# atomicarchitects/equiformer

Measured on NVIDIA H100. Metric: edges/sec fwd+bwd, QM9 Lmax=2 batch, higher is better.
Workload: dtype f32

## Files before the change

equiformer_b200/csrc/eqf_gemm_tf32x3.cu:

```cuda
#include <cuda.h>
#include <cuda_runtime.h>

#include <cstdint>
#include <cstdlib>
#include <mutex>
#include <string>

#include "eqf_common.cuh"
#include "eqf_tc.cuh"

namespace eqf {
namespace tf32x3 {

using namespace tc;

constexpr int BM = 128;
constexpr int BK = kKTile;
constexpr int kRowBytes = BK * 4;
constexpr int kThreads = 384;
constexpr int kConsumerWarps = 8, kConsumerThreads = kConsumerWarps * 32;
constexpr int kSmemBudget = 227 * 1024;
constexpr int kMaxStages = 8;

template <int BN>
struct Smem {
  static constexpr int kABytes = BM * kRowBytes;
  static constexpr int kBBytes = BN * kRowBytes;
  static constexpr int kStageBytes = kABytes + 2 * kBBytes;
  static constexpr int kStagesRaw = (kSmemBudget - 2048) / kStageBytes;
  static constexpr int kStages = kStagesRaw > kMaxStages ? kMaxStages : kStagesRaw;
  static_assert(kStages >= 2, "tile does not fit shared memory");
  static constexpr int kTotal = kStages * kStageBytes + 1024  + 1024 ;
};

struct Params {
  float* C;
  long long M, ldc;
  long long n_tiles;
  int n_blocks;
  int N, K;
};

template <int BN>
__global__ void __launch_bounds__(kThreads, 1)
gemm_tf32x3_kernel(const __grid_constant__ CUtensorMap map_a, const __grid_constant__ CUtensorMap map_bhi,
                   const __grid_constant__ CUtensorMap map_blo, Params p) {
  using S = Smem<BN>;
  constexpr int kStages = S::kStages;
  extern __shared__ uint8_t smem_raw[];
  uint8_t* smem = reinterpret_cast<uint8_t*>((reinterpret_cast<uintptr_t>(smem_raw) + 1023) & ~uintptr_t(1023));
  uint64_t* full = reinterpret_cast<uint64_t*>(smem + kStages * S::kStageBytes);
  uint64_t* empty = full + kStages;

  const int warp = threadIdx.x >> 5, lane = threadIdx.x & 31, wg = warp >> 2;
  const int k_tiles = (p.K + BK - 1) / BK;
  if (threadIdx.x == 0) {
    for (int s = 0; s < kStages; ++s) { mbar_init(&full[s], 1); mbar_init(&empty[s], kConsumerWarps); }
    asm volatile("fence.mbarrier_init.release.cluster;" ::: "memory");
  }
  __syncthreads();

  if (wg == 0) {
    reg_dealloc<40>();
    if (threadIdx.x == 0) {
      prefetch_map(&map_a); prefetch_map(&map_bhi); prefetch_map(&map_blo);
      int s = 0;
      uint32_t ph = 0;
      for (long long tile = blockIdx.x; tile < p.n_tiles; tile += gridDim.x) {
        const int m0 = (int)(tile / p.n_blocks) * BM;
        const int n0 = (int)(tile % p.n_blocks) * BN;
        for (int kt = 0; kt < k_tiles; ++kt) {
          mbar_wait_hint(&empty[s], ph ^ 1);
          uint8_t* st = smem + s * S::kStageBytes;
          mbar_expect_tx(&full[s], (uint32_t)S::kStageBytes);
          tma_load_2d(st, &map_a, kt * BK, m0, &full[s]);
          tma_load_2d(st + S::kABytes, &map_bhi, kt * BK, n0, &full[s]);
          tma_load_2d(st + S::kABytes + S::kBBytes, &map_blo, kt * BK, n0, &full[s]);
          if (++s == kStages) { s = 0; ph ^= 1; }
        }
      }
    }
  } else {
    reg_alloc<232>();
    const int row_wg = (wg - 1) * 64 + (warp & 3) * 16;
    int s = 0;
    uint32_t ph = 0;
    for (long long tile = blockIdx.x; tile < p.n_tiles; tile += gridDim.x) {
      const long long m0 = (tile / p.n_blocks) * BM;
      const int n0 = (int)(tile % p.n_blocks) * BN;
      float acc[BN / 2], part[BN / 2];
#pragma unroll
      for (int i = 0; i < BN / 2; ++i) acc[i] = 0.f;
      for (int kt = 0; kt < k_tiles; ++kt) {
        mbar_wait_hint(&full[s], ph);
        const uint32_t st = smem_u32(smem + s * S::kStageBytes);
        uint32_t hi[16], lo[16];
        load_a_split(st, row_wg, lane, hi, lo);
#pragma unroll
        for (int i = 0; i < BN / 2; ++i) part[i] = 0.f;
        mma_ktile_3xtf32<BN>(part, hi, lo, st + S::kABytes, st + S::kABytes + S::kBBytes);
        wgmma_wait<0>();
        __syncwarp();
        if (lane == 0) mbar_arrive(&empty[s]);
#pragma unroll
        for (int i = 0; i < BN / 2; ++i) acc[i] += part[i];
        if (++s == kStages) { s = 0; ph ^= 1; }
      }
      store_acc<BN>(acc, p.C, p.ldc, m0 + row_wg, p.M, n0, p.N, lane, false);
    }
  }
}

__global__ void split_kernel(const float* __restrict__ w, float* __restrict__ hi, float* __restrict__ lo, long long n) {
  for (long long i = (long long)blockIdx.x * blockDim.x + threadIdx.x; i < n; i += (long long)gridDim.x * blockDim.x) {
    const float v = w[i];
    const float h = tf32_rn(v);
    hi[i] = h;
    lo[i] = tf32_rn(v - h);
  }
}

__global__ void split_transpose_kernel(const float* __restrict__ w, long long ldw, float* __restrict__ hi,
                                       float* __restrict__ lo, long long N, long long K) {
  const long long n_el = N * K;
  for (long long i = (long long)blockIdx.x * blockDim.x + threadIdx.x; i < n_el; i += (long long)gridDim.x * blockDim.x) {
    const long long n = i / K, k = i - n * K;
    const float v = w[k * ldw + n];
    const float h = tf32_rn(v);
    hi[i] = h;
    lo[i] = tf32_rn(v - h);
  }
}

template <int BN>
static int launch(const CUtensorMap& ma, const CUtensorMap& mh, const CUtensorMap& ml, const Params& p, long long m_blocks,
                  int n_blocks, cudaStream_t s) {
  static std::once_flag once;
  static cudaError_t attr_err = cudaSuccess;
  std::call_once(once, [] {
    attr_err = cudaFuncSetAttribute(gemm_tf32x3_kernel<BN>, cudaFuncAttributeMaxDynamicSharedMemorySize, Smem<BN>::kTotal);
  });
  if (attr_err != cudaSuccess) return check_cuda(attr_err, "gemm_tf32x3 smem attribute");
  Params q = p;
  q.n_blocks = n_blocks;
  q.n_tiles = m_blocks * n_blocks;
  const long long sms = device_sms();
  const unsigned grid = (unsigned)(q.n_tiles < sms ? q.n_tiles : sms);
  gemm_tf32x3_kernel<BN><<<grid, kThreads, Smem<BN>::kTotal, s>>>(ma, mh, ml, q);
  return check_cuda(cudaGetLastError(), "gemm_tf32x3_kernel launch");
}

namespace wg {

constexpr int BKR = BK;
constexpr int kBoxBytes = BKR * 128;
constexpr int kMaxBN = 128;

struct WParams {
  float* out;
  long long R, rows_per_slice, K1;
  int N;
  int reduce;
};

template <int BN>
struct WSmem {
  static constexpr int kABytes = (BM / 32) * kBoxBytes;
  static constexpr int kGRawBytes = BKR * BN * 4;
  static constexpr int kGBytes = BN * kRowBytes;
  static constexpr int kStageBytes = kABytes + kGRawBytes + 2 * kGBytes;
  static constexpr int kStagesRaw = (kSmemBudget - 2048) / kStageBytes;
  static constexpr int kStages = kStagesRaw > kMaxStages ? kMaxStages : kStagesRaw;
  static_assert(kStages >= 2, "tile does not fit shared memory");
  static constexpr int kTotal = kStages * kStageBytes + 1024 + 1024;
};

__device__ __forceinline__ void load_at_split(uint32_t tile, int row0, int lane, uint32_t (&hi)[16], uint32_t (&lo)[16]) {
  const int g = row0 + (lane >> 2), t = lane & 3;
#pragma unroll
  for (int kb = 0; kb < BKR / 8; ++kb) {
#pragma unroll
    for (int q = 0; q < 4; ++q) {
      const int m = g + ((q & 1) ? 8 : 0);
      const int r = kb * 8 + t + ((q & 2) ? 4 : 0);
      const int c = m & 31;
      const uint32_t addr = tile + (uint32_t)(m >> 5) * kBoxBytes + (uint32_t)r * 128u + (uint32_t)((((c >> 2) ^ (r & 7)) << 4) + (c & 3) * 4);
      const float x = lds32(addr);
      const float h = tf32_rn_fast(x);
      hi[kb * 4 + q] = __float_as_uint(h);
      lo[kb * 4 + q] = __float_as_uint(tf32_rn_fast(x - h));
    }
  }
}

template <int BN>
__global__ void __launch_bounds__(kThreads, 1)
wgrad_tf32x3_kernel(const __grid_constant__ CUtensorMap map_a, const __grid_constant__ CUtensorMap map_g, WParams p) {
  using S = WSmem<BN>;
  constexpr int kStages = S::kStages;
  extern __shared__ uint8_t smem_raw[];
  uint8_t* smem = reinterpret_cast<uint8_t*>((reinterpret_cast<uintptr_t>(smem_raw) + 1023) & ~uintptr_t(1023));
  uint64_t* full = reinterpret_cast<uint64_t*>(smem + kStages * S::kStageBytes);
  uint64_t* empty = full + kStages;

  const int warp = threadIdx.x >> 5, lane = threadIdx.x & 31, wgi = warp >> 2;
  const int m0 = blockIdx.x * BM;
  const int n0 = blockIdx.y * BN;
  const long long r_begin = (long long)blockIdx.z * p.rows_per_slice;
  long long r_end = r_begin + p.rows_per_slice;
  if (r_end > p.R) r_end = p.R;
  const int k_tiles = (int)((r_end - r_begin + BKR - 1) / BKR);
  if (threadIdx.x == 0) {
    for (int s = 0; s < kStages; ++s) { mbar_init(&full[s], 1); mbar_init(&empty[s], kConsumerWarps); }
    asm volatile("fence.mbarrier_init.release.cluster;" ::: "memory");
  }
  __syncthreads();

  if (wgi == 0) {
    reg_dealloc<40>();
    if (threadIdx.x == 0) {
      prefetch_map(&map_a); prefetch_map(&map_g);
      for (int kt = 0; kt < k_tiles; ++kt) {
        const int s = kt % kStages;
        mbar_wait_hint(&empty[s], ((kt / kStages) & 1) ^ 1);
        uint8_t* st = smem + s * S::kStageBytes;
        const int r = (int)(r_begin + (long long)kt * BKR);
        mbar_expect_tx(&full[s], (uint32_t)(S::kABytes + S::kGRawBytes));
#pragma unroll
        for (int b = 0; b < BM / 32; ++b) tma_load_2d(st + b * kBoxBytes, &map_a, m0 + 32 * b, r, &full[s]);
        tma_load_2d(st + S::kABytes, &map_g, n0, r, &full[s]);
      }
    }
  } else {
    reg_alloc<232>();
    const int ct = threadIdx.x - 128;
    const int row_wg = (wgi - 1) * 64 + (warp & 3) * 16;
    float acc[BN / 2], part[BN / 2];
#pragma unroll
    for (int i = 0; i < BN / 2; ++i) acc[i] = 0.f;
    for (int kt = 0; kt < k_tiles; ++kt) {
      const int s = kt % kStages;
      mbar_wait_hint(&full[s], (kt / kStages) & 1);
      const uint32_t st = smem_u32(smem + s * S::kStageBytes);
      const uint32_t g_raw = st + S::kABytes, g_hi = g_raw + S::kGRawBytes, g_lo = g_hi + S::kGBytes;
      for (int i = ct; i < BN * (BKR / 4); i += kConsumerThreads) {
        const int n = i % BN, rq = i / BN;
        float4 v;
        v.x = lds32(g_raw + (uint32_t)((4 * rq + 0) * BN + n) * 4u);
        v.y = lds32(g_raw + (uint32_t)((4 * rq + 1) * BN + n) * 4u);
        v.z = lds32(g_raw + (uint32_t)((4 * rq + 2) * BN + n) * 4u);
        v.w = lds32(g_raw + (uint32_t)((4 * rq + 3) * BN + n) * 4u);
        float4 h;
        h.x = tf32_rn_fast(v.x); h.y = tf32_rn_fast(v.y); h.z = tf32_rn_fast(v.z); h.w = tf32_rn_fast(v.w);
        const uint32_t off = (uint32_t)n * 128u + (uint32_t)((rq ^ (n & 7)) << 4);
        sts128(g_hi + off, h);
        sts128(g_lo + off, make_float4(tf32_rn_fast(v.x - h.x), tf32_rn_fast(v.y - h.y), tf32_rn_fast(v.z - h.z),
                                       tf32_rn_fast(v.w - h.w)));
      }
      fence_async_smem();
      named_barrier(1, kConsumerThreads);
      uint32_t hi[16], lo[16];
      load_at_split(st, row_wg, lane, hi, lo);
#pragma unroll
      for (int i = 0; i < BN / 2; ++i) part[i] = 0.f;
      mma_ktile_3xtf32<BN>(part, hi, lo, g_hi, g_lo);
      wgmma_wait<0>();
      __syncwarp();
      if (lane == 0) mbar_arrive(&empty[s]);
#pragma unroll
      for (int i = 0; i < BN / 2; ++i) acc[i] += part[i];
    }
    float* out = p.reduce ? p.out : p.out + (long long)blockIdx.z * p.K1 * p.N;
    store_acc<BN>(acc, out, p.N, m0 + row_wg, p.K1, n0, p.N, lane, p.reduce != 0);
  }
}

struct Shape { int n_tile, n_tiles, m_tiles; long long slices, rows_per_slice; };

static Shape plan(long long R, long long K1, long long N) {
  Shape sh;
  sh.n_tiles = (int)((N + kMaxBN - 1) / kMaxBN);
  sh.n_tile = sh.n_tiles == 1 ? (int)((N + 31) & ~31LL) : kMaxBN;
  sh.m_tiles = (int)((K1 + BM - 1) / BM);
  const long long sms = device_sms();
  long long slices = sms / ((long long)sh.m_tiles * sh.n_tiles);
  if (slices < 1) slices = 1;
  long long rps = (R + slices - 1) / slices;
  if (rps < 64) rps = 64;
  rps = (rps + BKR - 1) / BKR * BKR;
  sh.rows_per_slice = rps;
  sh.slices = (R + rps - 1) / rps;
  return sh;
}

template <int BN>
static int launch(const CUtensorMap& ma, const CUtensorMap& mg, const WParams& p, const Shape& sh, cudaStream_t s) {
  static std::once_flag once;
  static cudaError_t attr_err = cudaSuccess;
  std::call_once(once, [] {
    attr_err = cudaFuncSetAttribute(wgrad_tf32x3_kernel<BN>, cudaFuncAttributeMaxDynamicSharedMemorySize, WSmem<BN>::kTotal);
  });
  if (attr_err != cudaSuccess) return check_cuda(attr_err, "wgrad_tf32x3 smem attribute");
  dim3 grid((unsigned)sh.m_tiles, (unsigned)sh.n_tiles, (unsigned)sh.slices);
  wgrad_tf32x3_kernel<BN><<<grid, kThreads, WSmem<BN>::kTotal, s>>>(ma, mg, p);
  return check_cuda(cudaGetLastError(), "wgrad_tf32x3_kernel launch");
}

}
}
}

using namespace eqf;

extern "C" int eqf_gemm_tf32x3(const float* A, const float* Bt, float* C, int64_t M, int64_t N, int64_t K, int64_t lda,
                               int64_t ldb, int64_t ldc, int32_t b_is_kn, float* split, void* stream) {
  using namespace eqf::tf32x3;
  if (M <= 0 || N <= 0) return EQF_OK;
  if (!A || !Bt || !C || !split) { set_error("eqf_gemm_tf32x3: null pointer"); return EQF_ERR_INVALID; }
  if (K <= 0) { set_error("eqf_gemm_tf32x3: K must be positive"); return EQF_ERR_INVALID; }
  if ((((uintptr_t)A | (uintptr_t)C | (uintptr_t)split) & 15) || ((K | lda | ldc) & 3) || lda < K || ldc < N ||
      ldb < (b_is_kn ? N : K)) {
    set_error("eqf_gemm_tf32x3: operands must be 16-byte aligned, K and leading dimensions multiples of 4");
    return EQF_ERR_INVALID;
  }
  if (K > 0x7fffffffLL || N > 0x7fffffffLL) { set_error("eqf_gemm_tf32x3: K / N too large"); return EQF_ERR_UNSUPPORTED; }
  cudaStream_t s = (cudaStream_t)stream;
  float* hi = split;
  float* lo = split + N * K;
  {
    const long long n = N * K;
    const unsigned blocks = (unsigned)((n + 255) / 256 < 1056 ? (n + 255) / 256 : 1056);
    if (b_is_kn) split_transpose_kernel<<<blocks, 256, 0, s>>>(Bt, ldb, hi, lo, N, K);
    else if (ldb == K) split_kernel<<<blocks, 256, 0, s>>>(Bt, hi, lo, n);
    else { set_error("eqf_gemm_tf32x3: Bt must be packed (ldb == K)"); return EQF_ERR_UNSUPPORTED; }
  }
  int rc = check_cuda(cudaGetLastError(), "split_kernel launch");
  if (rc != EQF_OK) return rc;
  const long long n_split = (N + 127) / 128;
  const long long per = (N + n_split - 1) / n_split;
  const int bn = per <= 32 ? 32 : per <= 64 ? 64 : per <= 96 ? 96 : 128;
  const int n_blocks = (int)((N + bn - 1) / bn);
  const long long m_blocks = (M + BM - 1) / BM;
  Params p;
  p.C = C; p.M = M; p.ldc = ldc; p.N = (int)N; p.K = (int)K;
  CUtensorMap ma, mh, ml;
  if ((rc = make_map_2d(&ma, A, M, K, lda, BM, BK)) != EQF_OK) return rc;
  if ((rc = make_map_2d(&mh, hi, N, K, K, bn, BK)) != EQF_OK) return rc;
  if ((rc = make_map_2d(&ml, lo, N, K, K, bn, BK)) != EQF_OK) return rc;
  switch (bn) {
    case 32: return launch<32>(ma, mh, ml, p, m_blocks, n_blocks, s);
    case 64: return launch<64>(ma, mh, ml, p, m_blocks, n_blocks, s);
    case 96: return launch<96>(ma, mh, ml, p, m_blocks, n_blocks, s);
    default: return launch<128>(ma, mh, ml, p, m_blocks, n_blocks, s);
  }
}

extern "C" int64_t eqf_gemm_tf32x3_wgrad_slices(int64_t R, int64_t K1, int64_t N) {
  if (R <= 0 || K1 <= 0 || N <= 0) return 0;
  return eqf::tf32x3::wg::plan(R, K1, N).slices;
}

static int wgrad_impl(const float* A, const float* G, float* out, bool reduce, int64_t R, int64_t K1, int64_t N,
                      int64_t lda, int64_t ldg, void* stream, const char* who) {
  using namespace eqf::tf32x3;
  if (R <= 0 || K1 <= 0 || N <= 0) return EQF_OK;
  if (!A || !G || !out) { set_error(std::string(who) + ": null pointer"); return EQF_ERR_INVALID; }
  if ((((uintptr_t)A | (uintptr_t)G | (uintptr_t)out) & 15) || ((K1 | N | lda | ldg) & 3) || lda < K1 || ldg < N) {
    set_error(std::string(who) + ": operands must be 16-byte aligned, dimensions multiples of 4");
    return EQF_ERR_INVALID;
  }
  if (R > 0x7fffffffLL || K1 > 0x7fffffffLL || N > 0x7fffffffLL) {
    set_error(std::string(who) + ": too many rows");
    return EQF_ERR_UNSUPPORTED;
  }
  const wg::Shape sh = wg::plan(R, K1, N);
  wg::WParams p;
  p.out = out; p.R = R; p.rows_per_slice = sh.rows_per_slice; p.K1 = K1; p.N = (int)N; p.reduce = reduce ? 1 : 0;
  CUtensorMap ma, mg;
  int rc;
  if ((rc = make_map_2d(&ma, A, R, K1, lda, wg::BKR, 32)) != EQF_OK) return rc;
  if ((rc = make_map_2d(&mg, G, R, N, ldg, wg::BKR, sh.n_tile, MapKind::kLinear)) != EQF_OK) return rc;
  cudaStream_t s = (cudaStream_t)stream;
  if (reduce && (rc = check_cuda(cudaMemsetAsync(out, 0, (size_t)K1 * N * sizeof(float), s), "wgrad memset")) != EQF_OK)
    return rc;
  if (sh.n_tile <= 32) return wg::launch<32>(ma, mg, p, sh, s);
  if (sh.n_tile <= 64) return wg::launch<64>(ma, mg, p, sh, s);
  if (sh.n_tile <= 96) return wg::launch<96>(ma, mg, p, sh, s);
  return wg::launch<128>(ma, mg, p, sh, s);
}

extern "C" int eqf_gemm_tf32x3_wgrad(const float* A, const float* G, float* partial, int64_t R, int64_t K1, int64_t N,
                                     int64_t lda, int64_t ldg, void* stream) {
  return wgrad_impl(A, G, partial, false, R, K1, N, lda, ldg, stream, "eqf_gemm_tf32x3_wgrad");
}

extern "C" int eqf_gemm_tf32x3_wgrad_accumulate(const float* A, const float* G, float* W, int64_t R, int64_t K1, int64_t N,
                                                int64_t lda, int64_t ldg, void* stream) {
  return wgrad_impl(A, G, W, true, R, K1, N, lda, ldg, stream, "eqf_gemm_tf32x3_wgrad_accumulate");
}
```

equiformer_b200/csrc/eqf_tc.cuh:

```cuda
#pragma once
#include <cuda.h>
#include <cuda_runtime.h>

#include <cstdint>
#include <string>

#include "eqf_common.cuh"

namespace eqf {
namespace tc {

__device__ __forceinline__ uint32_t smem_u32(const void* p) { return (uint32_t)__cvta_generic_to_shared(p); }

__device__ __forceinline__ void mbar_init(uint64_t* bar, uint32_t count) {
  asm volatile("mbarrier.init.shared::cta.b64 [%0], %1;" ::"r"(smem_u32(bar)), "r"(count));
}
__device__ __forceinline__ void mbar_arrive(uint64_t* bar) {
  asm volatile("mbarrier.arrive.shared::cta.b64 _, [%0];" ::"r"(smem_u32(bar)) : "memory");
}
__device__ __forceinline__ void mbar_expect_tx(uint64_t* bar, uint32_t bytes) {
  asm volatile("mbarrier.arrive.expect_tx.shared::cta.b64 _, [%0], %1;" ::"r"(smem_u32(bar)), "r"(bytes) : "memory");
}
__device__ __forceinline__ void mbar_wait(uint64_t* bar, uint32_t parity) {
  uint32_t done;
  do {
    asm volatile("{\n\t.reg .pred p;\n\tmbarrier.try_wait.parity.shared::cta.b64 p, [%1], %2;\n\tselp.u32 %0, 1, 0, p;\n\t}"
                 : "=r"(done) : "r"(smem_u32(bar)), "r"(parity) : "memory");
  } while (!done);
}
__device__ __forceinline__ void mbar_wait_hint(uint64_t* bar, uint32_t parity) {
  asm volatile(
      "{\n\t.reg .pred p;\n\t"
      "WAIT_%=:\n\t"
      "mbarrier.try_wait.parity.shared::cta.b64 p, [%0], %1, %2;\n\t"
      "@p bra DONE_%=;\n\t"
      "bra WAIT_%=;\n\t"
      "DONE_%=:\n\t}"
      ::"r"(smem_u32(bar)), "r"(parity), "r"(0x989680u) : "memory");
}
__device__ __forceinline__ void tma_load_2d(void* dst, const CUtensorMap* map, int c0, int c1, uint64_t* bar) {
  asm volatile("cp.async.bulk.tensor.2d.shared::cluster.global.mbarrier::complete_tx::bytes [%0], [%1, {%2, %3}], [%4];"
               ::"r"(smem_u32(dst)), "l"(reinterpret_cast<uint64_t>(map)), "r"(c0), "r"(c1), "r"(smem_u32(bar)) : "memory");
}
__device__ __forceinline__ void prefetch_map(const CUtensorMap* map) {
  asm volatile("prefetch.tensormap [%0];" ::"l"(reinterpret_cast<uint64_t>(map)) : "memory");
}
__device__ __forceinline__ void fence_async_smem() { asm volatile("fence.proxy.async.shared::cta;" ::: "memory"); }

__device__ __forceinline__ float tf32_rn(float x) {
  uint32_t r;
  asm("cvt.rna.tf32.f32 %0, %1;" : "=r"(r) : "f"(x));
  return __uint_as_float(r);
}
__device__ __forceinline__ float tf32_rn_fast(float x) {
  return __uint_as_float((__float_as_uint(x) + 0x1000u) & 0xffffe000u);
}

__device__ __forceinline__ float lds32(uint32_t addr) {
  float v;
  asm volatile("ld.shared.f32 %0, [%1];" : "=f"(v) : "r"(addr));
  return v;
}
__device__ __forceinline__ float4 lds128(uint32_t addr) {
  float4 v;
  asm volatile("ld.shared.v4.f32 {%0, %1, %2, %3}, [%4];" : "=f"(v.x), "=f"(v.y), "=f"(v.z), "=f"(v.w) : "r"(addr));
  return v;
}
__device__ __forceinline__ void sts128(uint32_t addr, const float4& v) {
  asm volatile("st.shared.v4.f32 [%0], {%1, %2, %3, %4};" ::"r"(addr), "f"(v.x), "f"(v.y), "f"(v.z), "f"(v.w) : "memory");
}

template <int N> __device__ __forceinline__ void reg_alloc() { asm volatile("setmaxnreg.inc.sync.aligned.u32 %0;" ::"n"(N)); }
template <int N> __device__ __forceinline__ void reg_dealloc() { asm volatile("setmaxnreg.dec.sync.aligned.u32 %0;" ::"n"(N)); }

__device__ __forceinline__ void named_barrier(int id, int threads) {
  asm volatile("bar.sync %0, %1;" ::"r"(id), "r"(threads) : "memory");
}

__device__ __forceinline__ uint64_t smem_desc_sw128(uint32_t addr) {
  return (uint64_t)((addr >> 4) & 0x3FFF) | (1ull << 16) | (64ull << 32) | (1ull << 62);
}
__device__ __forceinline__ void wgmma_fence() { asm volatile("wgmma.fence.sync.aligned;" ::: "memory"); }
__device__ __forceinline__ void wgmma_commit() { asm volatile("wgmma.commit_group.sync.aligned;" ::: "memory"); }
template <int N> __device__ __forceinline__ void wgmma_wait() { asm volatile("wgmma.wait_group.sync.aligned %0;" ::"n"(N) : "memory"); }

__device__ __forceinline__ void wgmma_rs_n32(float* d, const uint32_t* a, uint64_t b_desc) {
  asm volatile(
      "{\n\t.reg .pred p;\n\tsetp.ne.b32 p, 1, 0;\n\t"
      "wgmma.mma_async.sync.aligned.m64n32k8.f32.tf32.tf32 "
      "{%0, %1, %2, %3, %4, %5, %6, %7, %8, %9, %10, %11, %12, %13, %14, %15}, "
      "{%16, %17, %18, %19}, %20, p, 1, 1;\n\t}"
      : "+f"(d[0]), "+f"(d[1]), "+f"(d[2]), "+f"(d[3]), "+f"(d[4]), "+f"(d[5]), "+f"(d[6]), "+f"(d[7]),
        "+f"(d[8]), "+f"(d[9]), "+f"(d[10]), "+f"(d[11]), "+f"(d[12]), "+f"(d[13]), "+f"(d[14]), "+f"(d[15])
      : "r"(a[0]), "r"(a[1]), "r"(a[2]), "r"(a[3]), "l"(b_desc));
}
__device__ __forceinline__ void wgmma_rs_n64(float* d, const uint32_t* a, uint64_t b_desc) {
  asm volatile(
      "{\n\t.reg .pred p;\n\tsetp.ne.b32 p, 1, 0;\n\t"
      "wgmma.mma_async.sync.aligned.m64n64k8.f32.tf32.tf32 "
      "{%0, %1, %2, %3, %4, %5, %6, %7, %8, %9, %10, %11, %12, %13, %14, %15, "
      "%16, %17, %18, %19, %20, %21, %22, %23, %24, %25, %26, %27, %28, %29, %30, %31}, "
      "{%32, %33, %34, %35}, %36, p, 1, 1;\n\t}"
      : "+f"(d[0]), "+f"(d[1]), "+f"(d[2]), "+f"(d[3]), "+f"(d[4]), "+f"(d[5]), "+f"(d[6]), "+f"(d[7]),
        "+f"(d[8]), "+f"(d[9]), "+f"(d[10]), "+f"(d[11]), "+f"(d[12]), "+f"(d[13]), "+f"(d[14]), "+f"(d[15]),
        "+f"(d[16]), "+f"(d[17]), "+f"(d[18]), "+f"(d[19]), "+f"(d[20]), "+f"(d[21]), "+f"(d[22]), "+f"(d[23]),
        "+f"(d[24]), "+f"(d[25]), "+f"(d[26]), "+f"(d[27]), "+f"(d[28]), "+f"(d[29]), "+f"(d[30]), "+f"(d[31])
      : "r"(a[0]), "r"(a[1]), "r"(a[2]), "r"(a[3]), "l"(b_desc));
}

constexpr int kKTile = 32;

template <int N4>
__device__ __forceinline__ void load_a_split(uint32_t tile, int row0, int lane, uint32_t (&hi)[N4], uint32_t (&lo)[N4],
                                             int kb0 = 0) {
  static_assert(N4 % 4 == 0 && N4 <= 4 * (kKTile / 8), "whole 8-deep k-steps of one k-tile");
  const int g = row0 + (lane >> 2), t = lane & 3;
#pragma unroll
  for (int kb = 0; kb < N4 / 4; ++kb) {
#pragma unroll
    for (int q = 0; q < 4; ++q) {
      const int r = g + ((q & 1) ? 8 : 0);
      const int c = (kb0 + kb) * 8 + t + ((q & 2) ? 4 : 0);
      const float x = lds32(tile + (uint32_t)r * 128u + (uint32_t)((((c >> 2) ^ (r & 7)) << 4) + (c & 3) * 4));
      const float h = tf32_rn_fast(x);
      hi[kb * 4 + q] = __float_as_uint(h);
      lo[kb * 4 + q] = __float_as_uint(tf32_rn_fast(x - h));
    }
  }
}

template <int BN, int N4>
__device__ __forceinline__ void mma_ktile_3xtf32(float* acc, const uint32_t (&hi)[N4], const uint32_t (&lo)[N4], uint32_t b_hi,
                                                 uint32_t b_lo, int kb0 = 0) {
  static_assert(BN % 32 == 0 && BN >= 32 && BN <= 256, "BN must be a multiple of 32 up to 256");
  wgmma_fence();
#pragma unroll
  for (int kb = 0; kb < N4 / 4; ++kb) {
    const uint64_t adv = (uint64_t)(((kb0 + kb) * 32) >> 4);
#pragma unroll
    for (int j = 0; j < BN / 64; ++j) {
      const uint64_t dh = smem_desc_sw128(b_hi + (uint32_t)j * 8192u) + adv, dl = smem_desc_sw128(b_lo + (uint32_t)j * 8192u) + adv;
      wgmma_rs_n64(acc + 32 * j, &lo[kb * 4], dh);
      wgmma_rs_n64(acc + 32 * j, &hi[kb * 4], dl);
      wgmma_rs_n64(acc + 32 * j, &hi[kb * 4], dh);
    }
    if constexpr (BN % 64 == 32) {
      constexpr int j = BN / 64;
      const uint64_t dh = smem_desc_sw128(b_hi + (uint32_t)j * 8192u) + adv, dl = smem_desc_sw128(b_lo + (uint32_t)j * 8192u) + adv;
      wgmma_rs_n32(acc + 32 * j, &lo[kb * 4], dh);
      wgmma_rs_n32(acc + 32 * j, &hi[kb * 4], dl);
      wgmma_rs_n32(acc + 32 * j, &hi[kb * 4], dh);
    }
  }
  wgmma_commit();
}

__device__ __forceinline__ int acc_row(int i, int lane) { return (lane >> 2) + ((i >> 1) & 1) * 8; }
__device__ __forceinline__ int acc_col(int i, int lane) { return 8 * ((i & 31) >> 2) + 2 * (lane & 3) + (i & 1) + 64 * (i >> 5); }

template <int BN>
__device__ __forceinline__ void store_acc(const float* acc, float* C, long long ldc, long long row0, long long M, int col0, int N,
                                          int lane, bool add) {
#pragma unroll
  for (int i = 0; i < BN / 2; i += 2) {
    const long long r = row0 + acc_row(i, lane);
    const int c = col0 + acc_col(i, lane);
    if (r >= M || c >= N) continue;
    float* p = C + r * ldc + c;
    if (add) {
      atomicAdd(p, acc[i]);
      if (c + 1 < N) atomicAdd(p + 1, acc[i + 1]);
    } else if (c + 1 < N) {
      *reinterpret_cast<float2*>(p) = make_float2(acc[i], acc[i + 1]);
    } else {
      *p = acc[i];
    }
  }
}

typedef CUresult (*EncodeTiled)(CUtensorMap*, CUtensorMapDataType, cuuint32_t, void*, const cuuint64_t*, const cuuint64_t*,
                                const cuuint32_t*, const cuuint32_t*, CUtensorMapInterleave, CUtensorMapSwizzle,
                                CUtensorMapL2promotion, CUtensorMapFloatOOBfill);

static inline EncodeTiled encode_fn() {
  static EncodeTiled fn = [] {
    void* f = nullptr;
    cudaDriverEntryPointQueryResult q;
    if (cudaGetDriverEntryPoint("cuTensorMapEncodeTiled", &f, cudaEnableDefault, &q) != cudaSuccess) f = nullptr;
    return reinterpret_cast<EncodeTiled>(f);
  }();
  return fn;
}

enum class MapKind { kSwizzled, kLinear };

static inline int make_map_2d(CUtensorMap* map, const float* base, long long rows, long long cols, long long ld, int box_rows,
                              int box_cols, MapKind kind = MapKind::kSwizzled) {
  EncodeTiled enc = encode_fn();
  if (enc == nullptr) { set_error("cuTensorMapEncodeTiled is not available from the driver"); return EQF_ERR_CUDA; }
  cuuint64_t dims[2] = {(cuuint64_t)cols, (cuuint64_t)rows};
  cuuint64_t strides[1] = {(cuuint64_t)ld * sizeof(float)};
  cuuint32_t box[2] = {(cuuint32_t)box_cols, (cuuint32_t)box_rows};
  cuuint32_t estr[2] = {1, 1};
  const CUtensorMapSwizzle sw = kind == MapKind::kLinear ? CU_TENSOR_MAP_SWIZZLE_NONE : CU_TENSOR_MAP_SWIZZLE_128B;
  CUresult r = enc(map, CU_TENSOR_MAP_DATA_TYPE_FLOAT32, 2, const_cast<float*>(base), dims, strides, box, estr,
                   CU_TENSOR_MAP_INTERLEAVE_NONE, sw, CU_TENSOR_MAP_L2_PROMOTION_L2_128B, CU_TENSOR_MAP_FLOAT_OOB_FILL_NONE);
  if (r != CUDA_SUCCESS) { set_error("cuTensorMapEncodeTiled failed (code " + std::to_string((int)r) + ")"); return EQF_ERR_CUDA; }
  return EQF_OK;
}

static inline int device_sms() {
  int sms = 132, dev = 0;
  cudaGetDevice(&dev);
  cudaDeviceGetAttribute(&sms, cudaDevAttrMultiProcessorCount, dev);
  return sms;
}

}
}
```

Before: 1.265 million.

## Overlap A-operand split with in-flight WGMMA and store GEMM output via TMA

The consumer loop in the 3xTF32 GEMM is software-pipelined: it issues the WGMMAs for the current k-tile, then waits on and splits the next stage's A fragments into hi/lo registers while those MMAs run. The weight-gradient kernel gets the same treatment, with its G transpose-split moved ahead. Output tiles are staged in swizzled shared memory and written with TMA bulk stores, and wide n96/n128 WGMMA instructions plus scale-d=0 replace the explicit zeroing of the partial accumulator. In exchange the code carries double-buffered fragment registers, reserves shared memory for output staging (which may reduce pipeline stages), and adds more complex synchronisation.

```diff
diff --git a/equiformer_b200/csrc/eqf_gemm_tf32x3.cu b/equiformer_b200/csrc/eqf_gemm_tf32x3.cu
--- a/equiformer_b200/csrc/eqf_gemm_tf32x3.cu
+++ b/equiformer_b200/csrc/eqf_gemm_tf32x3.cu
@@ -27,29 +27,89 @@
   static constexpr int kABytes = BM * kRowBytes;
   static constexpr int kBBytes = BN * kRowBytes;
   static constexpr int kStageBytes = kABytes + 2 * kBBytes;
-  static constexpr int kStagesRaw = (kSmemBudget - 2048) / kStageBytes;
+  static constexpr int kOutBytes = 64 * BN * 4;
+  static constexpr int kStagesRaw = (kSmemBudget - 2048 - 2 * kOutBytes) / kStageBytes;
   static constexpr int kStages = kStagesRaw > kMaxStages ? kMaxStages : kStagesRaw;
   static_assert(kStages >= 2, "tile does not fit shared memory");
-  static constexpr int kTotal = kStages * kStageBytes + 1024  + 1024 ;
+  static constexpr int kTotal = kStages * kStageBytes + 2 * kOutBytes + 1024  + 1024 ;
 };
 
 struct Params {
-  float* C;
-  long long M, ldc;
   long long n_tiles;
   int n_blocks;
   int N, K;
 };
 
 template <int BN>
+__device__ __forceinline__ void stage_acc(const float* acc, uint32_t out, int row_w, int lane) {
+#pragma unroll
+  for (int i = 0; i < BN / 2; i += 2) {
+    const int r = row_w + acc_row(i, lane), c = acc_col(i, lane), cc = c & 31;
+    const uint32_t addr = out + (uint32_t)(c >> 5) * 8192u + (uint32_t)r * 128u + (uint32_t)((((cc >> 2) ^ (r & 7)) << 4) + (cc & 3) * 4);
+    asm volatile("st.shared.v2.f32 [%0], {%1, %2};" ::"r"(addr), "f"(acc[i]), "f"(acc[i + 1]) : "memory");
+  }
+}
+
+template <int BN>
+struct Consumer {
+  using S = Smem<BN>;
+  uint8_t* smem;
+  uint64_t *full, *empty;
+  const CUtensorMap* map_c;
+  uint32_t out;
+  long long tile, n_tiles;
+  int kt, k_tiles, n_blocks, s, row_w, row_wg, lane, wg;
+  uint32_t ph;
+  bool leader;
+  float acc[BN / 2], part[BN / 2];
+
+  __device__ __forceinline__ bool step(const uint32_t (&hc)[16], const uint32_t (&lc)[16], uint32_t (&hn)[16],
+                                       uint32_t (&ln)[16]) {
+    const uint32_t st = smem_u32(smem + s * S::kStageBytes);
+    mma_ktile_3xtf32<BN, true>(part, hc, lc, st + S::kABytes, st + S::kABytes + S::kBBytes);
+    const int s_cur = s;
+    const int kt_cur = kt;
+    const long long tile_cur = tile;
+    if (++s == S::kStages) { s = 0; ph ^= 1; }
+    if (++kt == k_tiles) { kt = 0; tile += gridDim.x; }
+    const bool more = tile < n_tiles;
+    if (more) {
+      mbar_wait_hint(&full[s], ph);
+      load_a_split(smem_u32(smem + s * S::kStageBytes), row_wg, lane, hn, ln);
+    }
+    wgmma_wait<0>();
+    __syncwarp();
+    if (lane == 0) mbar_arrive(&empty[s_cur]);
+#pragma unroll
+    for (int i = 0; i < BN / 2; ++i) acc[i] = kt_cur == 0 ? part[i] : acc[i] + part[i];
+    if (kt_cur == k_tiles - 1) {
+      if (leader) bulk_wait_read();
+      named_barrier(wg, 128);
+      stage_acc<BN>(acc, out, row_w, lane);
+      fence_async_smem();
+      named_barrier(wg, 128);
+      if (leader) {
+        const int m0 = (int)(tile_cur / n_blocks) * BM + (wg - 1) * 64;
+        const int n0 = (int)(tile_cur % n_blocks) * BN;
+#pragma unroll
+        for (int b = 0; b < BN / 32; ++b) tma_store_2d(map_c, n0 + 32 * b, m0, out + (uint32_t)b * 8192u);
+        bulk_commit();
+      }
+    }
+    return more;
+  }
+};
+
+template <int BN>
 __global__ void __launch_bounds__(kThreads, 1)
 gemm_tf32x3_kernel(const __grid_constant__ CUtensorMap map_a, const __grid_constant__ CUtensorMap map_bhi,
-                   const __grid_constant__ CUtensorMap map_blo, Params p) {
+                   const __grid_constant__ CUtensorMap map_blo, const __grid_constant__ CUtensorMap map_c, Params p) {
   using S = Smem<BN>;
   constexpr int kStages = S::kStages;
   extern __shared__ uint8_t smem_raw[];
   uint8_t* smem = reinterpret_cast<uint8_t*>((reinterpret_cast<uintptr_t>(smem_raw) + 1023) & ~uintptr_t(1023));
-  uint64_t* full = reinterpret_cast<uint64_t*>(smem + kStages * S::kStageBytes);
+  uint8_t* out_base = smem + kStages * S::kStageBytes;
+  uint64_t* full = reinterpret_cast<uint64_t*>(out_base + 2 * S::kOutBytes);
   uint64_t* empty = full + kStages;
 
   const int warp = threadIdx.x >> 5, lane = threadIdx.x & 31, wg = warp >> 2;
@@ -82,32 +142,21 @@
     }
   } else {
     reg_alloc<232>();
-    const int row_wg = (wg - 1) * 64 + (warp & 3) * 16;
-    int s = 0;
-    uint32_t ph = 0;
-    for (long long tile = blockIdx.x; tile < p.n_tiles; tile += gridDim.x) {
-      const long long m0 = (tile / p.n_blocks) * BM;
-      const int n0 = (int)(tile % p.n_blocks) * BN;
-      float acc[BN / 2], part[BN / 2];
-#pragma unroll
-      for (int i = 0; i < BN / 2; ++i) acc[i] = 0.f;
-      for (int kt = 0; kt < k_tiles; ++kt) {
-        mbar_wait_hint(&full[s], ph);
-        const uint32_t st = smem_u32(smem + s * S::kStageBytes);
-        uint32_t hi[16], lo[16];
-        load_a_split(st, row_wg, lane, hi, lo);
-#pragma unroll
-        for (int i = 0; i < BN / 2; ++i) part[i] = 0.f;
-        mma_ktile_3xtf32<BN>(part, hi, lo, st + S::kABytes, st + S::kABytes + S::kBBytes);
-        wgmma_wait<0>();
-        __syncwarp();
-        if (lane == 0) mbar_arrive(&empty[s]);
-#pragma unroll
-        for (int i = 0; i < BN / 2; ++i) acc[i] += part[i];
-        if (++s == kStages) { s = 0; ph ^= 1; }
-      }
-      store_acc<BN>(acc, p.C, p.ldc, m0 + row_wg, p.M, n0, p.N, lane, false);
-    }
+    if ((long long)blockIdx.x >= p.n_tiles) return;
+    Consumer<BN> c;
+    c.smem = smem; c.full = full; c.empty = empty; c.map_c = &map_c;
+    c.out = smem_u32(out_base + (wg - 1) * S::kOutBytes);
+    c.tile = blockIdx.x; c.n_tiles = p.n_tiles; c.kt = 0; c.k_tiles = k_tiles; c.n_blocks = p.n_blocks;
+    c.s = 0; c.ph = 0; c.lane = lane; c.wg = wg;
+    c.row_w = (warp & 3) * 16;
+    c.row_wg = (wg - 1) * 64 + c.row_w;
+    c.leader = (threadIdx.x & 127) == 0;
+    if (c.leader) prefetch_map(&map_c);
+    uint32_t h0[16], l0[16], h1[16], l1[16];
+    mbar_wait_hint(&full[0], 0);
+    load_a_split(smem_u32(smem), c.row_wg, lane, h0, l0);
+    while (c.step(h0, l0, h1, l1) && c.step(h1, l1, h0, l0)) {}
+    if (c.leader) bulk_wait();
   }
 }
 
@@ -133,8 +182,8 @@
 }
 
 template <int BN>
-static int launch(const CUtensorMap& ma, const CUtensorMap& mh, const CUtensorMap& ml, const Params& p, long long m_blocks,
-                  int n_blocks, cudaStream_t s) {
+static int launch(const CUtensorMap& ma, const CUtensorMap& mh, const CUtensorMap& ml, const CUtensorMap& mc, const Params& p,
+                  long long m_blocks, int n_blocks, cudaStream_t s) {
   static std::once_flag once;
   static cudaError_t attr_err = cudaSuccess;
   std::call_once(once, [] {
@@ -146,7 +195,7 @@
   q.n_tiles = m_blocks * n_blocks;
   const long long sms = device_sms();
   const unsigned grid = (unsigned)(q.n_tiles < sms ? q.n_tiles : sms);
-  gemm_tf32x3_kernel<BN><<<grid, kThreads, Smem<BN>::kTotal, s>>>(ma, mh, ml, q);
+  gemm_tf32x3_kernel<BN><<<grid, kThreads, Smem<BN>::kTotal, s>>>(ma, mh, ml, mc, q);
   return check_cuda(cudaGetLastError(), "gemm_tf32x3_kernel launch");
 }
 
@@ -235,14 +284,9 @@
     reg_alloc<232>();
     const int ct = threadIdx.x - 128;
     const int row_wg = (wgi - 1) * 64 + (warp & 3) * 16;
-    float acc[BN / 2], part[BN / 2];
-#pragma unroll
-    for (int i = 0; i < BN / 2; ++i) acc[i] = 0.f;
-    for (int kt = 0; kt < k_tiles; ++kt) {
-      const int s = kt % kStages;
-      mbar_wait_hint(&full[s], (kt / kStages) & 1);
-      const uint32_t st = smem_u32(smem + s * S::kStageBytes);
-      const uint32_t g_raw = st + S::kABytes, g_hi = g_raw + S::kGRawBytes, g_lo = g_hi + S::kGBytes;
+    auto transpose_split = [&](int s) {
+      const uint32_t g_raw = smem_u32(smem + s * S::kStageBytes) + S::kABytes, g_hi = g_raw + S::kGRawBytes,
+                     g_lo = g_hi + S::kGBytes;
       for (int i = ct; i < BN * (BKR / 4); i += kConsumerThreads) {
         const int n = i % BN, rq = i / BN;
         float4 v;
@@ -258,18 +302,35 @@
                                        tf32_rn_fast(v.w - h.w)));
       }
       fence_async_smem();
-      named_barrier(1, kConsumerThreads);
-      uint32_t hi[16], lo[16];
-      load_at_split(st, row_wg, lane, hi, lo);
-#pragma unroll
-      for (int i = 0; i < BN / 2; ++i) part[i] = 0.f;
-      mma_ktile_3xtf32<BN>(part, hi, lo, g_hi, g_lo);
+    };
+    float acc[BN / 2], part[BN / 2];
+    int kt = 0;
+    auto step = [&](const uint32_t (&hc)[16], const uint32_t (&lc)[16], uint32_t (&hn)[16], uint32_t (&ln)[16]) {
+      const int s = kt % kStages;
+      const uint32_t g_hi = smem_u32(smem + s * S::kStageBytes) + S::kABytes + S::kGRawBytes;
+      mma_ktile_3xtf32<BN, true>(part, hc, lc, g_hi, g_hi + S::kGBytes);
+      const bool more = kt + 1 < k_tiles;
+      if (more) {
+        const int s1 = (kt + 1) % kStages;
+        mbar_wait_hint(&full[s1], ((kt + 1) / kStages) & 1);
+        transpose_split(s1);
+        load_at_split(smem_u32(smem + s1 * S::kStageBytes), row_wg, lane, hn, ln);
+      }
       wgmma_wait<0>();
       __syncwarp();
       if (lane == 0) mbar_arrive(&empty[s]);
 #pragma unroll
-      for (int i = 0; i < BN / 2; ++i) acc[i] += part[i];
-    }
+      for (int i = 0; i < BN / 2; ++i) acc[i] = kt == 0 ? part[i] : acc[i] + part[i];
+      if (more) named_barrier(1, kConsumerThreads);
+      ++kt;
+      return more;
+    };
+    uint32_t h0[16], l0[16], h1[16], l1[16];
+    mbar_wait_hint(&full[0], 0);
+    transpose_split(0);
+    load_at_split(smem_u32(smem), row_wg, lane, h0, l0);
+    named_barrier(1, kConsumerThreads);
+    while (step(h0, l0, h1, l1) && step(h1, l1, h0, l0)) {}
     float* out = p.reduce ? p.out : p.out + (long long)blockIdx.z * p.K1 * p.N;
     store_acc<BN>(acc, out, p.N, m0 + row_wg, p.K1, n0, p.N, lane, p.reduce != 0);
   }
@@ -341,17 +402,19 @@
   const int bn = per <= 32 ? 32 : per <= 64 ? 64 : per <= 96 ? 96 : 128;
   const int n_blocks = (int)((N + bn - 1) / bn);
   const long long m_blocks = (M + BM - 1) / BM;
+  if (M > 0x7fffffffLL) { set_error("eqf_gemm_tf32x3: M too large"); return EQF_ERR_UNSUPPORTED; }
   Params p;
-  p.C = C; p.M = M; p.ldc = ldc; p.N = (int)N; p.K = (int)K;
-  CUtensorMap ma, mh, ml;
+  p.N = (int)N; p.K = (int)K;
+  CUtensorMap ma, mh, ml, mc;
   if ((rc = make_map_2d(&ma, A, M, K, lda, BM, BK)) != EQF_OK) return rc;
   if ((rc = make_map_2d(&mh, hi, N, K, K, bn, BK)) != EQF_OK) return rc;
   if ((rc = make_map_2d(&ml, lo, N, K, K, bn, BK)) != EQF_OK) return rc;
+  if ((rc = make_map_2d(&mc, C, M, N, ldc, 64, 32)) != EQF_OK) return rc;
   switch (bn) {
-    case 32: return launch<32>(ma, mh, ml, p, m_blocks, n_blocks, s);
-    case 64: return launch<64>(ma, mh, ml, p, m_blocks, n_blocks, s);
-    case 96: return launch<96>(ma, mh, ml, p, m_blocks, n_blocks, s);
-    default: return launch<128>(ma, mh, ml, p, m_blocks, n_blocks, s);
+    case 32: return launch<32>(ma, mh, ml, mc, p, m_blocks, n_blocks, s);
+    case 64: return launch<64>(ma, mh, ml, mc, p, m_blocks, n_blocks, s);
+    case 96: return launch<96>(ma, mh, ml, mc, p, m_blocks, n_blocks, s);
+    default: return launch<128>(ma, mh, ml, mc, p, m_blocks, n_blocks, s);
   }
 }
 
diff --git a/equiformer_b200/csrc/eqf_tc.cuh b/equiformer_b200/csrc/eqf_tc.cuh
--- a/equiformer_b200/csrc/eqf_tc.cuh
+++ b/equiformer_b200/csrc/eqf_tc.cuh
@@ -42,6 +42,13 @@
   asm volatile("cp.async.bulk.tensor.2d.shared::cluster.global.mbarrier::complete_tx::bytes [%0], [%1, {%2, %3}], [%4];"
                ::"r"(smem_u32(dst)), "l"(reinterpret_cast<uint64_t>(map)), "r"(c0), "r"(c1), "r"(smem_u32(bar)) : "memory");
 }
+__device__ __forceinline__ void tma_store_2d(const CUtensorMap* map, int c0, int c1, uint32_t src) {
+  asm volatile("cp.async.bulk.tensor.2d.global.shared::cta.bulk_group [%0, {%1, %2}], [%3];"
+               ::"l"(reinterpret_cast<uint64_t>(map)), "r"(c0), "r"(c1), "r"(src) : "memory");
+}
+__device__ __forceinline__ void bulk_commit() { asm volatile("cp.async.bulk.commit_group;" ::: "memory"); }
+__device__ __forceinline__ void bulk_wait_read() { asm volatile("cp.async.bulk.wait_group.read 0;" ::: "memory"); }
+__device__ __forceinline__ void bulk_wait() { asm volatile("cp.async.bulk.wait_group 0;" ::: "memory"); }
 __device__ __forceinline__ void prefetch_map(const CUtensorMap* map) {
   asm volatile("prefetch.tensormap [%0];" ::"l"(reinterpret_cast<uint64_t>(map)) : "memory");
 }
@@ -84,19 +91,21 @@
 __device__ __forceinline__ void wgmma_commit() { asm volatile("wgmma.commit_group.sync.aligned;" ::: "memory"); }
 template <int N> __device__ __forceinline__ void wgmma_wait() { asm volatile("wgmma.wait_group.sync.aligned %0;" ::"n"(N) : "memory"); }
 
+template <int kScaleD = 1>
 __device__ __forceinline__ void wgmma_rs_n32(float* d, const uint32_t* a, uint64_t b_desc) {
   asm volatile(
-      "{\n\t.reg .pred p;\n\tsetp.ne.b32 p, 1, 0;\n\t"
+      "{\n\t.reg .pred p;\n\tsetp.ne.b32 p, %21, 0;\n\t"
       "wgmma.mma_async.sync.aligned.m64n32k8.f32.tf32.tf32 "
       "{%0, %1, %2, %3, %4, %5, %6, %7, %8, %9, %10, %11, %12, %13, %14, %15}, "
       "{%16, %17, %18, %19}, %20, p, 1, 1;\n\t}"
       : "+f"(d[0]), "+f"(d[1]), "+f"(d[2]), "+f"(d[3]), "+f"(d[4]), "+f"(d[5]), "+f"(d[6]), "+f"(d[7]),
         "+f"(d[8]), "+f"(d[9]), "+f"(d[10]), "+f"(d[11]), "+f"(d[12]), "+f"(d[13]), "+f"(d[14]), "+f"(d[15])
-      : "r"(a[0]), "r"(a[1]), "r"(a[2]), "r"(a[3]), "l"(b_desc));
-}
+      : "r"(a[0]), "r"(a[1]), "r"(a[2]), "r"(a[3]), "l"(b_desc), "n"(kScaleD));
+}
+template <int kScaleD = 1>
 __device__ __forceinline__ void wgmma_rs_n64(float* d, const uint32_t* a, uint64_t b_desc) {
   asm volatile(
-      "{\n\t.reg .pred p;\n\tsetp.ne.b32 p, 1, 0;\n\t"
+      "{\n\t.reg .pred p;\n\tsetp.ne.b32 p, %37, 0;\n\t"
       "wgmma.mma_async.sync.aligned.m64n64k8.f32.tf32.tf32 "
       "{%0, %1, %2, %3, %4, %5, %6, %7, %8, %9, %10, %11, %12, %13, %14, %15, "
       "%16, %17, %18, %19, %20, %21, %22, %23, %24, %25, %26, %27, %28, %29, %30, %31}, "
@@ -105,7 +114,45 @@
         "+f"(d[8]), "+f"(d[9]), "+f"(d[10]), "+f"(d[11]), "+f"(d[12]), "+f"(d[13]), "+f"(d[14]), "+f"(d[15]),
         "+f"(d[16]), "+f"(d[17]), "+f"(d[18]), "+f"(d[19]), "+f"(d[20]), "+f"(d[21]), "+f"(d[22]), "+f"(d[23]),
         "+f"(d[24]), "+f"(d[25]), "+f"(d[26]), "+f"(d[27]), "+f"(d[28]), "+f"(d[29]), "+f"(d[30]), "+f"(d[31])
-      : "r"(a[0]), "r"(a[1]), "r"(a[2]), "r"(a[3]), "l"(b_desc));
+      : "r"(a[0]), "r"(a[1]), "r"(a[2]), "r"(a[3]), "l"(b_desc), "n"(kScaleD));
+}
+
+template <int kScaleD = 1>
+__device__ __forceinline__ void wgmma_rs_n96(float* d, const uint32_t* a, uint64_t b_desc) {
+  asm volatile(
+      "{\n\t.reg .pred p;\n\tsetp.ne.b32 p, %53, 0;\n\t"
+      "wgmma.mma_async.sync.aligned.m64n96k8.f32.tf32.tf32 "
+      "{%0, %1, %2, %3, %4, %5, %6, %7, %8, %9, %10, %11, %12, %13, %14, %15, "
+      "%16, %17, %18, %19, %20, %21, %22, %23, %24, %25, %26, %27, %28, %29, %30, %31, "
+      "%32, %33, %34, %35, %36, %37, %38, %39, %40, %41, %42, %43, %44, %45, %46, %47}, "
+      "{%48, %49, %50, %51}, %52, p, 1, 1;\n\t}"
+      : "+f"(d[0]), "+f"(d[1]), "+f"(d[2]), "+f"(d[3]), "+f"(d[4]), "+f"(d[5]), "+f"(d[6]), "+f"(d[7]),
+        "+f"(d[8]), "+f"(d[9]), "+f"(d[10]), "+f"(d[11]), "+f"(d[12]), "+f"(d[13]), "+f"(d[14]), "+f"(d[15]),
+        "+f"(d[16]), "+f"(d[17]), "+f"(d[18]), "+f"(d[19]), "+f"(d[20]), "+f"(d[21]), "+f"(d[22]), "+f"(d[23]),
+        "+f"(d[24]), "+f"(d[25]), "+f"(d[26]), "+f"(d[27]), "+f"(d[28]), "+f"(d[29]), "+f"(d[30]), "+f"(d[31]),
+        "+f"(d[32]), "+f"(d[33]), "+f"(d[34]), "+f"(d[35]), "+f"(d[36]), "+f"(d[37]), "+f"(d[38]), "+f"(d[39]),
+        "+f"(d[40]), "+f"(d[41]), "+f"(d[42]), "+f"(d[43]), "+f"(d[44]), "+f"(d[45]), "+f"(d[46]), "+f"(d[47])
+      : "r"(a[0]), "r"(a[1]), "r"(a[2]), "r"(a[3]), "l"(b_desc), "n"(kScaleD));
+}
+template <int kScaleD = 1>
+__device__ __forceinline__ void wgmma_rs_n128(float* d, const uint32_t* a, uint64_t b_desc) {
+  asm volatile(
+      "{\n\t.reg .pred p;\n\tsetp.ne.b32 p, %69, 0;\n\t"
+      "wgmma.mma_async.sync.aligned.m64n128k8.f32.tf32.tf32 "
+      "{%0, %1, %2, %3, %4, %5, %6, %7, %8, %9, %10, %11, %12, %13, %14, %15, "
+      "%16, %17, %18, %19, %20, %21, %22, %23, %24, %25, %26, %27, %28, %29, %30, %31, "
+      "%32, %33, %34, %35, %36, %37, %38, %39, %40, %41, %42, %43, %44, %45, %46, %47, "
+      "%48, %49, %50, %51, %52, %53, %54, %55, %56, %57, %58, %59, %60, %61, %62, %63}, "
+      "{%64, %65, %66, %67}, %68, p, 1, 1;\n\t}"
+      : "+f"(d[0]), "+f"(d[1]), "+f"(d[2]), "+f"(d[3]), "+f"(d[4]), "+f"(d[5]), "+f"(d[6]), "+f"(d[7]),
+        "+f"(d[8]), "+f"(d[9]), "+f"(d[10]), "+f"(d[11]), "+f"(d[12]), "+f"(d[13]), "+f"(d[14]), "+f"(d[15]),
+        "+f"(d[16]), "+f"(d[17]), "+f"(d[18]), "+f"(d[19]), "+f"(d[20]), "+f"(d[21]), "+f"(d[22]), "+f"(d[23]),
+        "+f"(d[24]), "+f"(d[25]), "+f"(d[26]), "+f"(d[27]), "+f"(d[28]), "+f"(d[29]), "+f"(d[30]), "+f"(d[31]),
+        "+f"(d[32]), "+f"(d[33]), "+f"(d[34]), "+f"(d[35]), "+f"(d[36]), "+f"(d[37]), "+f"(d[38]), "+f"(d[39]),
+        "+f"(d[40]), "+f"(d[41]), "+f"(d[42]), "+f"(d[43]), "+f"(d[44]), "+f"(d[45]), "+f"(d[46]), "+f"(d[47]),
+        "+f"(d[48]), "+f"(d[49]), "+f"(d[50]), "+f"(d[51]), "+f"(d[52]), "+f"(d[53]), "+f"(d[54]), "+f"(d[55]),
+        "+f"(d[56]), "+f"(d[57]), "+f"(d[58]), "+f"(d[59]), "+f"(d[60]), "+f"(d[61]), "+f"(d[62]), "+f"(d[63])
+      : "r"(a[0]), "r"(a[1]), "r"(a[2]), "r"(a[3]), "l"(b_desc), "n"(kScaleD));
 }
 
 constexpr int kKTile = 32;
@@ -129,7 +176,7 @@
   }
 }
 
-template <int BN, int N4>
+template <int BN, bool kFresh = false, int N4>
 __device__ __forceinline__ void mma_ktile_3xtf32(float* acc, const uint32_t (&hi)[N4], const uint32_t (&lo)[N4], uint32_t b_hi,
                                                  uint32_t b_lo, int kb0 = 0) {
   static_assert(BN % 32 == 0 && BN >= 32 && BN <= 256, "BN must be a multiple of 32 up to 256");
@@ -137,19 +184,36 @@
 #pragma unroll
   for (int kb = 0; kb < N4 / 4; ++kb) {
     const uint64_t adv = (uint64_t)(((kb0 + kb) * 32) >> 4);
-#pragma unroll
-    for (int j = 0; j < BN / 64; ++j) {
-      const uint64_t dh = smem_desc_sw128(b_hi + (uint32_t)j * 8192u) + adv, dl = smem_desc_sw128(b_lo + (uint32_t)j * 8192u) + adv;
-      wgmma_rs_n64(acc + 32 * j, &lo[kb * 4], dh);
-      wgmma_rs_n64(acc + 32 * j, &hi[kb * 4], dl);
-      wgmma_rs_n64(acc + 32 * j, &hi[kb * 4], dh);
-    }
-    if constexpr (BN % 64 == 32) {
-      constexpr int j = BN / 64;
-      const uint64_t dh = smem_desc_sw128(b_hi + (uint32_t)j * 8192u) + adv, dl = smem_desc_sw128(b_lo + (uint32_t)j * 8192u) + adv;
-      wgmma_rs_n32(acc + 32 * j, &lo[kb * 4], dh);
-      wgmma_rs_n32(acc + 32 * j, &hi[kb * 4], dl);
-      wgmma_rs_n32(acc + 32 * j, &hi[kb * 4], dh);
+    if constexpr (BN == 96 || BN == 128) {
+      const uint64_t dh = smem_desc_sw128(b_hi) + adv, dl = smem_desc_sw128(b_lo) + adv;
+      if constexpr (BN == 96) {
+        if (kFresh && kb == 0) wgmma_rs_n96<0>(acc, &lo[kb * 4], dh);
+        else wgmma_rs_n96(acc, &lo[kb * 4], dh);
+        wgmma_rs_n96(acc, &hi[kb * 4], dl);
+        wgmma_rs_n96(acc, &hi[kb * 4], dh);
+      } else {
+        if (kFresh && kb == 0) wgmma_rs_n128<0>(acc, &lo[kb * 4], dh);
+        else wgmma_rs_n128(acc, &lo[kb * 4], dh);
+        wgmma_rs_n128(acc, &hi[kb * 4], dl);
+        wgmma_rs_n128(acc, &hi[kb * 4], dh);
+      }
+    } else {
+#pragma unroll
+      for (int j = 0; j < BN / 64; ++j) {
+        const uint64_t dh = smem_desc_sw128(b_hi + (uint32_t)j * 8192u) + adv, dl = smem_desc_sw128(b_lo + (uint32_t)j * 8192u) + adv;
+        if (kFresh && kb == 0) wgmma_rs_n64<0>(acc + 32 * j, &lo[kb * 4], dh);
+        else wgmma_rs_n64(acc + 32 * j, &lo[kb * 4], dh);
+        wgmma_rs_n64(acc + 32 * j, &hi[kb * 4], dl);
+        wgmma_rs_n64(acc + 32 * j, &hi[kb * 4], dh);
+      }
+      if constexpr (BN % 64 == 32) {
+        constexpr int j = BN / 64;
+        const uint64_t dh = smem_desc_sw128(b_hi + (uint32_t)j * 8192u) + adv, dl = smem_desc_sw128(b_lo + (uint32_t)j * 8192u) + adv;
+        if (kFresh && kb == 0) wgmma_rs_n32<0>(acc + 32 * j, &lo[kb * 4], dh);
+        else wgmma_rs_n32(acc + 32 * j, &lo[kb * 4], dh);
+        wgmma_rs_n32(acc + 32 * j, &hi[kb * 4], dl);
+        wgmma_rs_n32(acc + 32 * j, &hi[kb * 4], dh);
+      }
     }
   }
   wgmma_commit();
```

After: 1.311 million (median of 6 runs). 3.7% higher.
